# alphafox02/iridium-sniffer

Hardware: AMD Instinct MI355X
Metric: IQ Msamples/s end-to-end (detect->demod), 10 MHz cf32 (higher is better)
Workload: dtype f32

## Files before the change

### iridium-sniffer_amd/csrc/api.cpp

```cpp
#include <stdarg.h>
#include "pipeline.hpp"

namespace irdmh {

extern "C" int irdm_set_option(irdm_pipeline_t *p, const char *key, int value)
{
    if (!p || !key) return -1;
    pipeline_enter(p);
    if (!strcmp(key, "keep_frame_samples")) { p->keep_frame_samples = value; return 0; }
    if (!strcmp(key, "packed_records")) { p->packed_records = value; return 0; }
    if (!strcmp(key, "parsed_records")) { p->parsed_records = value; return 0; }
    if (!strcmp(key, "frame_records")) { p->frame_records = value; return 0; }
    if (!strcmp(key, "chunk_marks")) { p->chunk_marks = value ? 1 : 0; if (!value) p->st.q_marks.clear(); return 0; }
    if (!strcmp(key, "group_member")) { p->in_group = value != 0; return 0; }
    if (!strcmp(key, "spectrum_frames")) {
        if (value < 0 || value > (1 << 20) || p->in_group || p->st.begin_no != 0) return -1;
        return spectrum_configure(p, value);
    }
    if (!strcmp(key, "input_stats")) {
        if (p->in_group || p->st.begin_no != p->st.end_no) return -1;
        return input_stats_configure(p, value);
    }
    if (!strcmp(key, "symbol_clock")) {
        if (p->in_group || p->st.begin_no != p->st.end_no) return -1;
        return symbol_clock_configure(p, value);
    }
    if (!strcmp(key, "decode_frames")) { p->decode_frames = value; return 0; }
    if (!strcmp(key, "decode_ida")) { p->decode_ida = value; return 0; }
    if (!strcmp(key, "detect_only")) { p->detect_only = value; return 0; }
    if (!strcmp(key, "fir_order") || !strcmp(key, "simd_order")) { p->fir_order = value ? 1 : 0; return 0; }
    if (!strcmp(key, "host_cfo")) { p->dev_cfo = p->dev_cfo_ok && value == 0; return 0; }
    if (!strcmp(key, "scan_mode")) { p->scan_mode = value; return 0; }
    if (!strcmp(key, "kernel_clock")) { p->kernel_clock = value != 0; return 0; }
    if (!strcmp(key, "rot_prebuild")) {
        if (value) return p->rot_pre_runs ? 0 : rot_prebuild(p);
        return p->rot_pre_runs ? rot_arena_reset(p, (long long)std::min(p->P.n, 1024) * p->rot_runs) : 0;
    }
    if (!strcmp(key, "band_timeline")) { p->band_tune.timeline = value != 0; return 0; }
    if (!strcmp(key, "fir_generic")) { p->fir_generic = value != 0; return 0; }
    if (!strcmp(key, "post_generic")) { p->post_generic = value != 0; return 0; }
    if (!strcmp(key, "k1_lists")) { p->k1_lists = value; return 0; }
    if (!strcmp(key, "band_first")) { p->band_first = value < 0 ? 0 : value > kBandRounds ? kBandRounds : value; return 0; }
    if (!strcmp(key, "band_spec")) { p->band_spec_opt = value != 0; return 0; }
    if (!strcmp(key, "band_selfcheck")) { p->band_tune.selfcheck = value; return 0; }
    if (!strcmp(key, "rot_pool_rows")) {
        if (value < 1 || value > p->P.n) return -1;
        return rot_arena_reset(p, (long long)value * p->rot_runs);
    }
    if (!strcmp(key, "scratch_outputs")) {
        if (value < 16) return -1;
        for (int i = 0; i < p->n_bc; i++)
            if (p->bc[i].st.n != 0) return -1;
        IRDM_HIP_CHECK(hipDeviceSynchronize());
        for (int i = 0; i < p->n_bc; i++) {
            BatchCtx &b = p->bc[i];
            float2 *d2 = dev_alloc<float2>((size_t)value), *l2 = dev_alloc<float2>(lpf_alloc((size_t)value));
            if (!d2 || !l2) return -1;
            (void)hipFree(b.d_dec);
            (void)hipFree(b.d_lpf);
            b.d_dec = d2;
            b.d_lpf = l2;
            b.dec_cap = (size_t)value;
            if (!b.owns_buffers) { p->d_dec = d2; p->d_lpf = l2; }
// ... 390 lines not shown
```

### iridium-sniffer_amd/csrc/chain.cpp

```cpp
#include "pipeline.hpp"

namespace irdmh {

SampleSource make_source(const irdm_pipeline *p, const void *chunk, uint64_t c0, uint64_t c1)
{
    SampleSource s;
    s.chunk = chunk;
    s.chunk_start = chunk ? c0 : ~0ull;
    s.chunk_end = c1;
    s.ring = p->d_ring;
    s.ring_len = p->ring_len;
    s.ref_ring = p->ref_ring;
    s.fmt = p->dev_fmt;
    s.n_cu = p->n_cu;
    return s;
}

int ring_guard(irdm_pipeline *p, uint64_t a0, uint64_t a1, hipStream_t st)
{
    const uint64_t L = p->ring_len;
    if (a1 <= a0 || L == 0) return 0;
    for (int i = 0; i < p->n_bc; i++) {
        const BatchCtx &b = p->bc[i];
        if (b.st.n <= 0 || b.st.ring_hi <= b.st.ring_lo) continue;
// ... 307 lines not shown
                p->rot_build_gen[(size_t)bin] = p->rot_gen[me] + 1;
            }
    }
    int n_new = 0;
    for (int bin : p->rot_touched) {
        const int from = p->rot_len_h[(size_t)bin], to = p->rot_want[(size_t)bin];
        if (from == 0) p->rot_rows_used++;
        b.hp_rot_new[n_new++] = int4{ bin, from, to, p->rot_blocks_used };
        p->rot_blocks_used += (to - from) / kRotRun;
        p->stat_rot_ckpts += (uint64_t)(to - from);
        p->rot_len_h[(size_t)bin] = to;
        p->rot_want[(size_t)bin] = 0;
        p->rot_build_ctx[(size_t)bin] = me;
        p->rot_build_gen[(size_t)bin] = p->rot_gen[me] + 1;
    }
    p->rot_gen[me]++;
    p->stat_rot_builds++;
    p->stat_rot_rows += (uint64_t)n_new;
    if (launch_copy_words(b.d_rot_new, b.hp_rot_new_dev, sizeof(int4) * (size_t)n_new, st) != 0) return -1;
    if (launch_rotator_rows(p->d_rot_incr, p->d_rot_table, p->rot_runs, b.d_rot_new, n_new, p->d_rot_slot, st) != 0) return -1;
    IRDM_HIP_CHECK(hipEventRecord(b.ev_rot, st));
    return wait_for(wait_mask & ~wait_first);
}

int bursts_enqueue(irdm_pipeline *p, BatchCtx &b, const SampleSource &src, const GoneBurst *gone_list, int nb)
{
    const DetParams &P = p->P;
    const int fs = p->cfg.sample_rate;
    b.st.n = nb;
    b.st.recs.assign(nb, irdm_burst_t());
    size_t n_tiles = 0, dec_need = 0;
    int max_dec_len = 0;
    const int fir_aligned = p->ring_len % 8 == 0 && p->ref_ring % 8 == 0 && (src.chunk_start == ~0ull || src.chunk_start % 8 == 0);
    const int tile_out = fir_tile_out(p->decim, fir_aligned, p->fir_generic, p->fir_order);
    for (int i = 0; i < nb; i++) {
        const GoneBurst &g = gone_list[i];
        irdm_burst_t &r = b.st.recs[i];
        r.id = g.id; r.start = g.start; r.stop = g.stop; r.last_active = g.last_active;
        r.center_bin = g.center_bin;
        r.peak_rel = g.peak_rel; r.base_sum = g.base_sum;
        r.magnitude = 10.0f * log10f(g.peak_rel * kHistory * 1.72f);
        if (r.magnitude > p->st.peak_signal_db) p->st.peak_signal_db = r.magnitude;
        r.noise = 10.0f * log10f(g.base_sum / kHistory / ((float)P.n * P.n) / 1.72f /
                                 ((float)fs / P.n));
        r.num_samples = g.stop + (uint64_t)P.pre_len - g.start;
        uint64_t e = (g.stop + (uint64_t)P.n + p->feed_block - 1) / p->feed_block * p->feed_block;
        r.avail_end = std::min<uint64_t>(e, src.chunk_end);

        BurstWork &w = b.hp_work[i];
        memset(&w, 0, sizeof(w));
        w.start = g.start;
        w.avail_end = r.avail_end;
        w.center_bin = g.center_bin;
        int n = r.num_samples > (uint64_t)(2 * 1024 * 1024) ? 2 * 1024 * 1024 : (int)r.num_samples;
        if ((size_t)n > p->l_cap) {
            fprintf(stderr, "irdm_hip: burst window %d exceeds l_cap %zu\n", n, p->l_cap);
            return -1;
        }
        w.n = n;
        w.dec_len = 0;
        w.drop_reason = 0;
        if (r.num_samples < 100) {
            w.drop_reason = 1;
        } else {
            int n_out = (n - p->in_ntaps + 1) / p->decim;
            if (n_out < 0) n_out = 0;
            w.dec_len = n_out;
            if (n_out < 100) w.drop_reason = 2;
        }
        w.tile_base = (int32_t)n_tiles;
        w.dec_off = (int32_t)dec_need;
        if (!w.drop_reason) {
            max_dec_len = std::max(max_dec_len, w.dec_len);
            n_tiles += (size_t)(w.dec_len + tile_out - 1) / tile_out;
            dec_need += ((size_t)w.dec_len + 15) & ~(size_t)15;
        }
    }
    b.st.ring_lo = b.st.ring_hi = 0;
    if (p->detect_only || nb == 0) return 0;
    {
        uint64_t lo = ~0ull, hi = 0;
        for (int i = 0; i < nb; i++) {
            const BurstWork &w = b.hp_work[i];
            if (w.drop_reason) continue;
            const uint64_t back = w.start + (uint64_t)w.n > w.avail_end ? p->ref_ring : 0;
            lo = std::min(lo, w.start > back ? w.start - back : 0);
            hi = std::max(hi, w.start + (uint64_t)w.n);
        }
        if (lo < hi) { b.st.ring_lo = lo; b.st.ring_hi = hi; }
    }
    if (dec_need > p->stat_scratch_peak) p->stat_scratch_peak = dec_need;
    if (dec_need > b.dec_cap) {
        const size_t cap2 = std::max(dec_need, 2 * b.dec_cap);
        if (cap2 > (size_t)0x7fffffff) {
            fprintf(stderr, "irdm_hip: %zu decimated samples in a batch of %d bursts\n", dec_need, nb);
            return -1;
        }
        float2 *d2 = dev_alloc<float2>(cap2), *l2 = dev_alloc<float2>(lpf_alloc(cap2));
        if (!d2 || !l2) {
            if (d2) (void)hipFree(d2);
            if (l2) (void)hipFree(l2);
            fprintf(stderr, "irdm_hip: no memory for %zu decimated samples per batch\n", cap2);
            return -1;
        }
        p->scratch_retired.push_back(b.d_dec);
        p->scratch_retired.push_back(b.d_lpf);
        b.d_dec = d2;
        b.d_lpf = l2;
        b.dec_cap = cap2;
        if (!b.owns_buffers) { p->d_dec = d2; p->d_lpf = l2; }
        p->stat_scratch_grows++;
    }
    const bool tile_list = fir_needs_tile_list(p->decim, fir_aligned, p->fir_generic) != 0;
    if (n_tiles > b.tiles_cap) {
        if (b.d_tiles) p->tiles_retired.push_back(b.d_tiles);
        if (b.hp_tiles) p->tiles_host_retired.push_back(b.hp_tiles);
        b.hp_tiles = nullptr;
        b.tiles_cap = n_tiles * 2;
        b.d_tiles = dev_alloc<FirTile>((b.tiles_cap + 1) * kFirTileUnits);
        if (!b.owns_buffers) p->d_tiles = b.d_tiles;
        if (!b.d_tiles ||
            hipHostMalloc(reinterpret_cast<void **>(&b.hp_tiles), sizeof(FirTile) * b.tiles_cap, hipHostMallocDefault) != hipSuccess)
            return -1;
        p->stat_tiles_grows++;
    }
    if (tile_list) {
        n_tiles = 0;
        for (int i = 0; i < nb; i++) {
            const BurstWork &w = b.hp_work[i];
            if (!w.drop_reason)
                for (int o = 0; o < w.dec_len; o += tile_out) b.hp_tiles[n_tiles++] = FirTile{ i, o };
        }
    }
    hipStream_t st = b.stream;
    if (rot_rows_prepare(p, b, nb, st) != 0) return -1;
    if (launch_copy_words(b.d_work, b.hp_work_dev, sizeof(BurstWork) * nb, st) != 0) return -1;
    if (tile_list && n_tiles && launch_copy_words(b.d_tiles, b.hp_tiles, sizeof(FirTile) * n_tiles, st) != 0) return -1;
    IRDM_HIP_CHECK(hipEventRecord(b.ev[0], st));
    if (launch_fir_decimate(src, b.d_work, nb, b.d_tiles, b.tiles_cap, (int)n_tiles, p->decim, p->d_in_taps,
                            p->d_fir_off, p->d_rot_incr, p->d_rot_table, p->rot_runs, b.d_dec, st,
                            p->kclk_fir((int)(&b - p->bc)), p->d_rot_slot, p->fir_order, p->fir_generic) != 0)
        return -1;
    IRDM_HIP_CHECK(hipEventRecord(b.ev[1], st));
    if (launch_downmix_post1(b.d_work, nb, max_dec_len, b.d_dec, b.d_lpf, box_of(b.d_lpf, b.dec_cap), p->d_noise_taps,
                             p->noise_ntaps, p->d_start_taps, p->start_ntaps, p->search_depth,
                             p->pre_start, p->d_cfo_window, p->d_tw4096, p->dev_cfo ? nullptr : b.hp_work_dev, st,
                             p->kclk_fir((int)(&b - p->bc)), p->fir_order, p->post_generic) != 0)
        return -1;
    CfoStep cfo;
    cfo.on_device = p->dev_cfo ? 1 : 0;
    cfo.n_fft = P.n;
    cfo.sample_rate = fs;
    cfo.out_rate = p->out_rate;
    cfo.center_frequency = p->cfg.center_frequency;
    b.cfo_on_device = p->dev_cfo;
    if (!p->dev_cfo) {
        IRDM_HIP_CHECK(hipEventRecord(b.ev_cfo, st));
        b.cfo_seq++;
        {
            std::lock_guard<std::mutex> lk(p->cfo_mu);
            p->cfo_jobs.push_back(&b);
        }
        p->cfo_cv.notify_one();
        if (launch_wait_host_flag(b.hp_flag_dev, b.cfo_seq, b.hp_flag_dev + 1, st) != 0) return -1;
    }
    if (launch_downmix_post2(b.d_work, nb, b.d_lpf, p->d_rrc_taps, p->rrc_ntaps,
                             p->d_tw2048, p->d_dl_fft, p->d_ul_fft, p->dl_len, p->ul_len, p->sps,
                             b.d_rrc_ws, b.d_frames, p->dev_cfo ? nullptr : b.hp_work_dev, cfo, st, p->fir_order, p->post_generic) != 0)
        return -1;
    IRDM_HIP_CHECK(hipEventRecord(b.ev[2], st));
    b.packed = (p->packed_records || p->parsed_records || p->frame_records) && !p->decode_frames && !p->decode_ida &&
               !p->keep_frame_samples;
    b.parsed = b.packed && p->parsed_records;
    b.framed = b.packed && p->frame_records;
// ... 218 lines not shown
```

### iridium-sniffer_amd/csrc/downmix.hip

```cpp
#include <algorithm>
#include <cstdio>
#include "common.hpp"
#include "types.hpp"
#include "kernels.hpp"
#include "burst_src.hpp"
#include "libm_port.hpp"

namespace irdm {

#include "fir_fma.inc"

__global__ void rotator_rows_kernel(const float2 *__restrict__ incr, float2 *__restrict__ table, int n_runs,
                                    const int4 *__restrict__ news, int n_new, int *__restrict__ runs_all)
{
    const int i = blockIdx.x * blockDim.x + threadIdx.x;
    if (i >= n_new) return;
    const int bin = news[i].x, from = news[i].y, to = news[i].z, block0 = news[i].w;
    const float2 inc = incr[bin];
    int *runs = runs_all + (size_t)bin * n_runs;
    float2 ph = make_float2(1.0f, 0.0f);
    if (from > 0) {
        ph = table[(size_t)runs[(from - 1) / kRotRun] * kRotRun + (from - 1) % kRotRun];
#pragma unroll
        for (int u = 0; u < kRotSeg; u++) ph = cmul(ph, inc);
// ... 175 lines not shown
    g.avail_end = w->avail_end;
    g.ring_pos = g.a_tile % ring_len;
    const int cb = w->center_bin;
    const float2 inc = rot_incr[cb];
    g.inc_re = inc.x;
    g.inc_im = inc.y;
    {
        const int c0 = g.s0 / kRotSeg, r0 = c0 / kRotRun;
        const int *runs = rot_slot + (size_t)cb * n_ckpt;
        const int b0 = runs[r0];
        int b1 = r0 + 1 < n_ckpt ? runs[r0 + 1] : b0;
        if (b1 < 0) b1 = b0;
        g.ck_index = (uint64_t)b0 * kRotRun + (uint64_t)(c0 % kRotRun);
        g.ck_wrap = kRotRun - c0 % kRotRun;
        g.ck_index2 = (uint64_t)b1 * kRotRun;
    }
    g.out_base = (int64_t)w->dec_off + o0;
    g.stale_pos = (g.ring_pos + ring_len - ref_ring % ring_len) % ring_len;
    g.pad = 0;
    geom[t] = g;
}

int fir_tile_row(int decim)
{
    int r = kFirTileOut + kFirTaps / decim + 2;
    while ((r & 15) != 1) r++;
    return r;
}

static bool fir_reg_path(int decim, int aligned, int generic) { return !generic && aligned && fir_reg_supported(decim); }

int fir_needs_tile_list(int decim, int aligned, int generic) { return fir_reg_path(decim, aligned, generic) ? 0 : 1; }

int fir_tile_out(int decim, int aligned, int generic, int order)
{
    if (!fir_reg_path(decim, aligned, generic)) return kFirTileOut;
    return order ? fir_fma_tile_out(decim) : fir_reg_tile_out(decim);
}

int launch_fir_decimate(const SampleSource &src, const BurstWork *work, int n_bursts, FirTile *tiles, size_t tiles_cap,
                        int n_tiles, int decim, const float *taps, const int *tap_off, const float2 *rot_incr,
                        const float2 *rot_table, int n_ckpt, float2 *dec,
                        hipStream_t stream, unsigned long long *kclk, const int *rot_slot, int order, int generic)
{
    if (n_tiles <= 0) return 0;
    const int aligned = src.ring_len % 8 == 0 && src.ref_ring % 8 == 0 && (src.chunk_start == ~0ull || src.chunk_start % 8 == 0);
    if (fir_reg_path(decim, aligned, generic) && tiles_cap >= (size_t)n_tiles) {
        FirGeom *geom = reinterpret_cast<FirGeom *>(tiles + tiles_cap);
        hipLaunchKernelGGL(fir_geom_kernel, dim3((n_tiles + 255) / 256), dim3(256), 0, stream, work, n_bursts, n_tiles, decim,
                           order ? fir_fma_tile_out(decim) : fir_reg_tile_out(decim), src.ring_len, src.ref_ring, rot_incr, n_ckpt,
                           geom, rot_slot);
        return (order ? launch_fir_fma(src, geom, n_tiles, decim, taps, rot_table, dec, stream, kclk)
                      : launch_fir_reg(src, geom, n_tiles, decim, taps, rot_table, dec, stream, kclk)) == 0 ? 0 : -1;
    }
    const int row = fir_tile_row(decim);
    const size_t lds = sizeof(float2) * (size_t)row * decim;
    if (lds > 160 * 1024) return -1;
    (void)hipFuncSetAttribute((const void *)fir_decimate_kernel,
                              hipFuncAttributeMaxDynamicSharedMemorySize, (int)lds);
    hipLaunchKernelGGL(fir_decimate_kernel, dim3(n_tiles), dim3(kFirTileOut), lds, stream, src, work,
                       tiles, decim, row, taps, tap_off, rot_incr, rot_table, n_ckpt, dec, order, rot_slot);
    return hipGetLastError() == hipSuccess ? 0 : -1;
}

__global__ void copy_words_kernel(uint32_t *__restrict__ dst, const uint32_t *__restrict__ src, size_t n)
{
    for (size_t i = blockIdx.x * (size_t)blockDim.x + threadIdx.x; i < n; i += (size_t)gridDim.x * blockDim.x)
        __hip_atomic_store(dst + i, __hip_atomic_load(src + i, __ATOMIC_RELAXED, __HIP_MEMORY_SCOPE_SYSTEM),
                           __ATOMIC_RELAXED, __HIP_MEMORY_SCOPE_SYSTEM);
    __threadfence_system();
}

__global__ void gone_export_kernel(const DetState *__restrict__ st, const uint32_t *__restrict__ gone, int cap,
                                   uint32_t *__restrict__ hp_gone, uint32_t *__restrict__ hp_hdr,
                                   const uint32_t *__restrict__ ctl, uint32_t *__restrict__ hp_ctl, int ctl_words)
{
    gone_export_body(st, gone, cap, hp_gone, hp_hdr, ctl, hp_ctl, ctl_words, (int)gridDim.x);
}

int launch_gone_export(const DetState *st, const GoneBurst *gone, int cap, GoneBurst *hp_gone, uint32_t *hp_hdr,
                       const void *ctl, void *hp_ctl, int ctl_bytes, hipStream_t stream)
{
    hipLaunchKernelGGL(gone_export_kernel, dim3(32), dim3(256), 0, stream, st, reinterpret_cast<const uint32_t *>(gone), cap,
// ... 744 lines not shown
```

### iridium-sniffer_amd/csrc/fir_reg.hip

```cpp
#include <cstdio>
#include "common.hpp"
#include "types.hpp"
#include "kernels.hpp"
#include "burst_src.hpp"

#ifndef IRDM_FIR_KCLK
#define IRDM_FIR_KCLK 1
#endif

namespace irdm {

#include "fir_mac.inc"

constexpr int kFirStrip = 3;

template <int M>
struct FirR {
    static constexpr int NR = kFirTaps / M;
    static constexpr int REM = kFirTaps - NR * M;
    static_assert(M % 8 == 0 && NR < 63 && REM >= 1, "geometry");
};

int fir_reg_supported(int decim) { return decim == 40 || decim == 48; }

// ... 220 lines not shown
            __builtin_amdgcn_sched_barrier(0);
            mac_rest(tb, H);
        }
        shift();
        {
            constexpr int P0 = REM >= H ? H : 0;
            if constexpr (REM >= H) {
                mac_head(ta, 0);
                mac_rest(ta, 0);
            }
            const uint64_t *t = taps64 + (NR * M + P0) / 2;
#pragma unroll
            for (int gq = 0; gq < (REM - P0) / 8; gq++)
                fir_mac2x8(acc[0], acc[1], &y[0][P0 + 8 * gq], &y[1][P0 + 8 * gq], t + 4 * gq);
#pragma unroll
            for (int p = P0 + (REM - P0) / 8 * 8; p < REM; p++) {
                const float tq = taps[NR * M + p];
                acc[0] = acc[0] + y[0][p] * tq;
                acc[1] = acc[1] + y[1][p] * tq;
            }
        }
#pragma unroll
        for (int j = 0; j < 2; j++) {
            const int q = 128 * d + 64 * j + lane - NR;
            if (q >= 0 && q < g.n_out) dec[g.out_base + q] = make_float2(acc[j].x, acc[j].y);
        }
    }
    }
    if (IRDM_FIR_KCLK) kclk_leave(kclk);
}

#include "fir_fma.inc"

int fir_fma_tile_out(int decim) { return 128 - kFirTaps / decim; }

template <int M, int FMT>
__device__ __forceinline__ void fir_fetch_column(const SampleSource &src, const FirGeom &g, int cr, int n_cols, v2f *y)
{
    const bool needed = cr < n_cols;
    const int k0 = needed ? cr * M : 0;
    const uint64_t a0 = g.a_tile + (uint64_t)k0;
    uint64_t rp = g.ring_pos + (uint64_t)k0;
    if (rp >= src.ring_len) rp -= src.ring_len;
    const bool in_chunk = a0 >= src.chunk_start;
    const bool simple = a0 + M <= g.avail_end && (in_chunk || (a0 + M <= src.chunk_start && rp + M <= src.ring_len));
    if (__builtin_amdgcn_ballot_w64(needed && !simple) == 0) {
        const void *base = in_chunk ? src.chunk : src.ring;
        const size_t idx = !needed ? 0 : in_chunk ? (size_t)(a0 - src.chunk_start) : (size_t)rp;
#pragma unroll
        for (int i = 0; i < M / 8; i++) load_piece<FMT>(base, idx + 8 * i, &y[8 * i]);
    } else {
        uint64_t rs = g.stale_pos + (uint64_t)k0;
        if (rs >= src.ring_len) rs -= src.ring_len;
#pragma unroll
        for (int i = 0; i < M / 8; i++) {
            const uint64_t a = a0 + 8 * i;
            v2f xn[8], xs[8];
#pragma unroll
            for (int u = 0; u < 8; u++) xn[u] = xs[u] = v2f{ 0.0f, 0.0f };
            if (needed && a < g.avail_end) {
                uint64_t p = rp + 8 * i;
                if (p >= src.ring_len) p -= src.ring_len;
                if (a >= src.chunk_start) load_piece<FMT>(src.chunk, (size_t)(a - src.chunk_start), xn);
                else load_piece<FMT>(src.ring, (size_t)p, xn);
            }
            if (needed && a + 8 > g.avail_end && a >= src.ref_ring) {
                const uint64_t as = a - src.ref_ring;
                uint64_t p = rs + 8 * i;
                if (p >= src.ring_len) p -= src.ring_len;
                if (as >= src.chunk_start) load_piece<FMT>(src.chunk, (size_t)(as - src.chunk_start), xs);
                else load_piece<FMT>(src.ring, (size_t)p, xs);
            }
#pragma unroll
            for (int u = 0; u < 8; u++) y[8 * i + u] = (a + u < g.avail_end) ? xn[u] : xs[u];
        }
    }
}

template <int M, int FMT>
__global__ __launch_bounds__(64) __attribute__((amdgpu_waves_per_eu(2, 2))) void fir_decimate_kernel_f(
    SampleSource src, const FirGeom *__restrict__ geom, const float *__restrict__ taps,
    const float2 *__restrict__ rot_table, float2 *__restrict__ dec, int n_tiles, unsigned long long *__restrict__ kclk)
{
    using R = FirR<M>;
    constexpr int NR = R::NR, REM = R::REM;
    constexpr int VT = REM - 1;
    static_assert(NR % 2 == 0, "rows are unrolled in pairs (the accumulator sets swap names)");
    static_assert(M % 4 == 0 && VT % 8 == 0 && (kFirTaps - 1) % 4 == 0, "tap k -> accumulator k % 4 = (k % M) % 4; one tap left over");
    const int lane = threadIdx.x;
    kclk_enter(kclk);
#pragma unroll 1
    for (int tile = blockIdx.x; tile < n_tiles;) {
        const int tile_next = tile + (int)gridDim.x;
        const FirGeom g = geom[tile];
        tile = tile_next;
        const int n_cols = g.n_out + NR;
        const v2f inc = { g.inc_re, g.inc_im };
        const uint64_t *taps64 = reinterpret_cast<const uint64_t *>(taps);
        v2f y[2][M];
#pragma unroll
        for (int j = 0; j < 2; j++) fir_fetch_column<M, FMT>(src, g, 2 * lane + j, n_cols, y[j]);
        {
            v2f ph[2];
#pragma unroll
            for (int j = 0; j < 2; j++) {
                const int cr = 2 * lane + j;
                const int k0 = cr < n_cols ? cr * M : 0;
                const float2 c = rot_table[fir_ck(g, k0 / kRotSeg)];
                ph[j] = v2f{ c.x, c.y };
            }
            if (M % kRotSeg != 0) {
                static_assert(M % kRotSeg == 0 || M % kRotSeg == 8, "a column starts on a checkpoint or 8 samples behind one");
                v2f pw = ph[1];
#pragma unroll
                for (int u = 0; u < 8; u++) pw = cmul_pk(pw, inc);
                if (2 * lane + 1 < n_cols) ph[1] = pw;
            }
#pragma unroll
            for (int p = 0; p < M; p++) {
                v2f r0, r1, n0, n1;
                cmul_pk2(r0, y[0][p], ph[0], r1, y[1][p], ph[1]);
                cmul_pk2(n0, ph[0], inc, n1, ph[1], inc);
                y[0][p] = r0;
                y[1][p] = r1;
                ph[0] = n0;
                ph[1] = n1;
            }
        }
        const v2f zero = { 0.0f, 0.0f };
        v2f X[4] = { zero, zero, zero, zero }, Y[4] = { zero, zero, zero, zero };
        constexpr int H = M / 2;
        static_assert(H == 20 || H == 24, "half rows of 8 + 8 + 4 or 8 + 8 + 8 taps");
        uint64_t ta[H / 2], tb[H / 2];
        auto request = [&](uint64_t (&t)[H / 2], int tap0) {
#pragma unroll
            for (int i = 0; i < H / 2; i++) t[i] = taps64[tap0 / 2 + i];
        };
        auto half_rest = [&](v2f (&xa)[4], v2f (&xb)[4], const uint64_t *t, int p0) {
            fir_fma2x8(xa, xb, &y[0][p0 + 8], &y[1][p0 + 8], t + 4);
            if constexpr (H == 24) fir_fma2x8(xa, xb, &y[0][p0 + 16], &y[1][p0 + 16], t + 8);
            else fir_fma2x4(xa, xb, &y[0][p0 + 16], &y[1][p0 + 16], t + 8);
        };
        auto row = [&](v2f (&xa)[4], v2f (&xb)[4], int r, int next_tap0) {
            fir_fma2x8(xa, xb, &y[0][0], &y[1][0], ta);
            __builtin_amdgcn_sched_barrier(0);
            request(tb, r * M + H);
            __builtin_amdgcn_sched_barrier(0);
            half_rest(xa, xb, ta, 0);
            fir_fma2x8(xa, xb, &y[0][H], &y[1][H], tb);
            __builtin_amdgcn_sched_barrier(0);
            request(ta, next_tap0);
            __builtin_amdgcn_sched_barrier(0);
            half_rest(xa, xb, tb, H);
        };
        auto shift = [&](v2f (&x)[4]) {
#pragma unroll
            for (int j = 0; j < 4; j++) {
                x[j].x = lane_shr1(x[j].x);
                x[j].y = lane_shr1(x[j].y);
            }
        };
        request(ta, 0);
#pragma unroll 1
        for (int rp = 0; rp < NR / 2; rp++) {
            row(X, Y, 2 * rp, (2 * rp + 1) * M);
            shift(Y);
            row(Y, X, 2 * rp + 1, (2 * rp + 2 < NR || VT >= H) ? (2 * rp + 2) * M : 0);
            shift(X);
        }
        if constexpr (VT > 0) {
            static_assert(VT < H || VT == H + 8, "VT = 32 at M = 48");
            if constexpr (VT >= H) {
                fir_fma2x8(X, Y, &y[0][0], &y[1][0], ta);
                half_rest(X, Y, ta, 0);
                const uint64_t *t = taps64 + (NR * M + H) / 2;
                fir_fma2x8(X, Y, &y[0][H], &y[1][H], t);
            } else {
                const uint64_t *t = taps64 + (NR * M) / 2;
#pragma unroll
                for (int gq = 0; gq < VT / 8; gq++) fir_fma2x8(X, Y, &y[0][8 * gq], &y[1][8 * gq], t + 4 * gq);
            }
        }
        {
            const float tq = taps[kFirTaps - 1];
            const v2f sa = (X[0] + X[2]) + (X[1] + X[3]), sb = (Y[0] + Y[2]) + (Y[1] + Y[3]);
            const v2f oa = sa + y[0][VT] * tq, ob = sb + y[1][VT] * tq;
            const int qa = 2 * lane - NR, qb = qa + 1;
            if (qa >= 0 && qa < g.n_out) dec[g.out_base + qa] = make_float2(oa.x, oa.y);
            if (qb >= 0 && qb < g.n_out) dec[g.out_base + qb] = make_float2(ob.x, ob.y);
        }
    }
    kclk_leave(kclk);
}

template <int M>
static int launch_fir_f_fmt(const SampleSource &src, const FirGeom *geom, int n_tiles, const float *taps,
                            const float2 *rot_table, float2 *dec, hipStream_t stream, unsigned long long *kclk)
{
    const int n_cu = src.n_cu > 0 ? src.n_cu : 256;
    const int grid = 7 * n_cu < n_tiles ? 7 * n_cu : n_tiles;
    if (src.fmt == 2) hipLaunchKernelGGL((fir_decimate_kernel_f<M, 2>), dim3(grid), dim3(64), 0, stream, src, geom, taps, rot_table, dec, n_tiles, kclk);
    else if (src.fmt == 1) hipLaunchKernelGGL((fir_decimate_kernel_f<M, 1>), dim3(grid), dim3(64), 0, stream, src, geom, taps, rot_table, dec, n_tiles, kclk);
    else if (src.fmt == 3) hipLaunchKernelGGL((fir_decimate_kernel_f<M, 3>), dim3(grid), dim3(64), 0, stream, src, geom, taps, rot_table, dec, n_tiles, kclk);
    else if (src.fmt == 4) hipLaunchKernelGGL((fir_decimate_kernel_f<M, 4>), dim3(grid), dim3(64), 0, stream, src, geom, taps, rot_table, dec, n_tiles, kclk);
    else if (src.fmt == 0) hipLaunchKernelGGL((fir_decimate_kernel_f<M, 0>), dim3(grid), dim3(64), 0, stream, src, geom, taps, rot_table, dec, n_tiles, kclk);
    else if (src.fmt == 6) hipLaunchKernelGGL((fir_decimate_kernel_f<M, 6>), dim3(grid), dim3(64), 0, stream, src, geom, taps, rot_table, dec, n_tiles, kclk);
    else if (src.fmt == 8) hipLaunchKernelGGL((fir_decimate_kernel_f<M, 8>), dim3(grid), dim3(64), 0, stream, src, geom, taps, rot_table, dec, n_tiles, kclk);
    else if (src.fmt == 9) hipLaunchKernelGGL((fir_decimate_kernel_f<M, 9>), dim3(grid), dim3(64), 0, stream, src, geom, taps, rot_table, dec, n_tiles, kclk);
    else return -1;
    return hipGetLastError() == hipSuccess ? 0 : -1;
}

int launch_fir_fma(const SampleSource &src, const FirGeom *geom, int n_tiles, int decim, const float *taps,
                   const float2 *rot_table, float2 *dec, hipStream_t stream, unsigned long long *kclk)
{
    if (src.ring_len % 8 != 0 || src.ref_ring % 8 != 0 || (src.chunk_start != ~0ull && src.chunk_start % 8 != 0)) return 1;
    switch (decim) {
    case 40: return launch_fir_f_fmt<40>(src, geom, n_tiles, taps, rot_table, dec, stream, kclk);
    case 48: return launch_fir_f_fmt<48>(src, geom, n_tiles, taps, rot_table, dec, stream, kclk);
    default: return 1;
    }
}
// ... 34 lines not shown
```

### iridium-sniffer_amd/csrc/kernels.hpp

```cpp
#pragma once
#include <hip/hip_runtime.h>
#include <vector>
#include "types.hpp"

namespace irdm {

int launch_fft_mag_lists(int log_n, int fmt, const void *iq, const float *window, const float2 *tw, float *mag,
                         int n_frames, const float *pre, unsigned *counts, ListEntry *entries, int cap,
                         hipStream_t stream, unsigned long long *kclk, int order);
int launch_prefilter_threshold(const float *sum, float thr, float *pre, int n, hipStream_t stream);
int launch_fft_mag(int log_n, int fmt, const void *iq, const float *window, const float2 *tw,
                   float *mag, int n_frames, hipStream_t stream, unsigned long long *kclk, int order);
int launch_detect_scan(const DetParams &P, DetState *st, float *sum, float *hist, const float *mag,
                       int n_frames, GoneBurst *gone, int gone_cap, PeakCand *cand_a,
                       PeakCand *cand_b, hipStream_t stream);

struct ZeroRegions {
    static constexpr int kMax = 8;
    uint32_t *ptr[kMax];
    uint32_t words[kMax];
    int n = 0;
    bool add(void *p, size_t bytes)
    {
        if (!p || n >= kMax || bytes % 4 != 0 || bytes / 4 > 0xffffffffull) return false;
// ... 67 lines not shown
    int sum_restart = 1;
};
int band_list_cap(int n);
int band_scan_supported(const DetParams &D, BandParams *out, int n_frames, uint64_t idx0);
size_t band_work_bytes(int n, size_t max_chunk, bool spec = false);
int band_work_carve(BandWork *W, void *base, int n, size_t max_chunk, bool spec = false);
int launch_band_spec(const DetParams &D, BandWork S, DetState *st_spec, const float *sum_src, int n_frames, uint64_t idx0,
                     const unsigned *counts, const ListEntry *entries, int have_prev, hipStream_t stream, const BandTune &tune);
int launch_band_scan(const DetParams &D, BandWork W, DetState *st, float *sum, float *hist, const float *mag,
                     int n_frames, uint64_t idx0, const unsigned *counts, const ListEntry *entries, const float *pre,
                     float *smin, GoneBurst *gone, int gone_cap, int round_begin, int round_end, GoneBurst *hp_gone,
                     uint32_t *hp_hdr, void *hp_ctl, int hp_cap, int chained, int tl_sel, hipStream_t stream,
                     const BandTune &tune, const uint32_t *gate_flag = nullptr, uint32_t gate_seq = 0, uint32_t *gate_err = nullptr,
                     const void *gate_src = nullptr, size_t gate_bytes = 0,
                     const BandWork *spec = nullptr, hipEvent_t sums_done = nullptr);
constexpr int kBandTlSlots = 32;
int launch_prefilter_lists(const float *sum, float thr, float *pre, const float *smin, const float *mag, int n,
                           unsigned *counts, ListEntry *entries, int n_frames, int cap, hipStream_t stream);

struct SampleSource {
    const void *chunk;
    uint64_t chunk_start;
    uint64_t chunk_end;
    const void *ring;
    uint64_t ring_len;
    uint64_t ref_ring;
    int fmt;
    int n_cu;
};

int launch_rotator_rows(const float2 *incr, float2 *table, int n_runs, const int4 *news, int n_new, int *runs, hipStream_t stream);
int fir_tile_row(int decim);
int fir_reg_supported(int decim);
int fir_fma_tile_out(int decim);
int fir_reg_tile_out(int decim);
int launch_fir_fma(const SampleSource &src, const FirGeom *geom, int n_tiles, int decim, const float *taps,
                   const float2 *rot_table, float2 *dec, hipStream_t stream, unsigned long long *kclk = nullptr);
int launch_fir_reg(const SampleSource &src, const FirGeom *geom, int n_tiles, int decim, const float *taps,
                   const float2 *rot_table, float2 *dec, hipStream_t stream, unsigned long long *kclk = nullptr);
int fir_tile_out(int decim, int aligned, int generic, int order);
int fir_needs_tile_list(int decim, int aligned, int generic);
int launch_fir_decimate(const SampleSource &src, const BurstWork *work, int n_bursts, FirTile *tiles, size_t tiles_cap,
                        int n_tiles, int decim, const float *taps, const int *tap_off, const float2 *rot_incr,
                        const float2 *rot_table, int n_ckpt, float2 *dec,
                        hipStream_t stream, unsigned long long *kclk,
                        const int *rot_slot, int order, int generic);
int launch_kclk_fold(unsigned long long *kclk, hipStream_t stream);
int launch_gone_export(const DetState *st, const GoneBurst *gone, int cap, GoneBurst *hp_gone, uint32_t *hp_hdr,
                       const void *ctl, void *hp_ctl, int ctl_bytes, hipStream_t stream);
int launch_copy_to_host(void *dst, const void *src, size_t bytes, hipStream_t stream);
int launch_copy2_to_host(void *dst_a, const void *src_a, size_t bytes_a, void *dst_b, const void *src_b, size_t bytes_b,
                         hipStream_t stream);
int launch_copy_words(void *dst, const void *src, size_t bytes, hipStream_t stream);
int launch_wait_host_flag(const uint32_t *flag, uint32_t seq, uint32_t *err, hipStream_t stream);
int launch_gather_burst(const SampleSource &src, uint64_t start, uint64_t avail_end, int n,
                        float2 *out, hipStream_t stream);
int launch_downmix_post1(BurstWork *work, int n_bursts, int max_dec_len, float2 *dec,
                         float2 *lpf, float *box, const float *noise_taps, int noise_ntaps,
                         const float *start_taps, int start_ntaps, int search_depth, int pre_start,
                         const float *cfo_window, const float2 *tw4096, BurstWork *hp_work, hipStream_t stream,
                         unsigned long long *kclk,
                         int order, int generic);
struct CfoStep {
    int on_device;
    int n_fft, sample_rate, out_rate;
    double center_frequency;
};
int launch_downmix_post2(BurstWork *work, int n_bursts, const float2 *lpf,
                         const float *rrc_taps, int rrc_ntaps, const float2 *tw2048,
                         const float2 *dl_fft, const float2 *ul_fft, int dl_len, int ul_len,
                         float sps, float2 *rrc_ws, float2 *frames, const BurstWork *hp_work, const CfoStep &cfo,
                         hipStream_t stream, int order, int generic);
int launch_sincosf_probe(const float *x, size_t n, float *re, float *im, hipStream_t stream);

int launch_ida_decode(const DemodOut *frames, int n_frames, const int2 *syn_da, const int2 *syn_l1, const int2 *syn_l2,
                      const int2 *syn_l3, int use_llr, const int *n_bits, const int *direction, IdaOut *out,
                      hipStream_t stream);
int launch_frame_decode(const DemodOut *frames, int n_frames, const int2 *syn_ra, const int2 *syn_hdr, int use_llr,
                        const int *n_bits, DecodedOut *out, hipStream_t stream);
// ... 46 lines not shown
```

### iridium-sniffer_amd/csrc/pipeline.hpp

```cpp
#pragma once
#include <math.h>
#include <stdlib.h>
#include <string.h>
#include <time.h>
#include <errno.h>
#include <sys/stat.h>
#include <algorithm>
#include <deque>
#include <new>
#include <vector>
#include <thread>
#include <mutex>
#include <condition_variable>
#include "../../include/irdm_hip.h"
#include "common.hpp"
#include "host_design.hpp"
#include "kernels.hpp"
#include "libm_port.hpp"
#include "band_core.hpp"
#include "types.hpp"
#include "record_queues.hpp"
#include "input_stats.hpp"
#include "symbol_clock.hpp"

// ... 149 lines not shown

struct irdm_pipeline {
    irdm_config_t cfg;
    StreamState st;
    DetParams P;
    int dev_fmt;
    size_t bps;
    int feed_block, decim, out_rate;
    bool dev_cfo;
    bool dev_cfo_ok;
    float sps;
    uint64_t ref_ring, ring_len;
    size_t l_cap;
    int n_ckpt, dec_stride, burst_cap, gone_cap;
    size_t max_chunk;
    int search_depth, pre_start;
    int in_ntaps, noise_ntaps, start_ntaps, rrc_ntaps, dl_len, ul_len;

    hipStream_t stream;
    hipStream_t bstream;
    hipStream_t stream2;
    int bstream_prio;
    hipStream_t sstream;
    hipEvent_t ev_scan_in, ev_scan_out;
    int band_spec_opt = 1;
    void *d_band_spec = nullptr;
    BandWork band_spec = {};
    DetState *d_state_spec = nullptr;
    hipStream_t stream_spec = nullptr;
    hipEvent_t ev_sums1 = nullptr;
    hipEvent_t ev_spec_done = nullptr;
    uint64_t stat_spec_passes = 0, stat_spec_scans = 0, stat_sum_restarts = 0;
    int fir_order = 1;
    int fir_generic = 0;
    int post_generic = 0;
    irdm::BandTune band_tune;
    hipEvent_t ev[10];

    float *d_window, *d_hist, *d_sum, *d_mag;
    float2 *d_tw, *d_tw4096, *d_tw2048, *d_dl_fft, *d_ul_fft, *d_rot_incr, *d_rot_table;
    DetState *d_state;
    GoneBurst *d_gone;
    PeakCand *d_cand_a, *d_cand_b;
    void *d_ring, *d_stage;
    float *d_in_taps, *d_noise_taps, *d_start_taps, *d_rrc_taps, *d_cfo_window;
    int *d_fir_off;
    BurstWork *d_work;
    FirTile *d_tiles;
    size_t tiles_cap;
    float2 *d_dec, *d_lpf, *d_rrc_ws, *d_frames, *d_demod_ws, *d_probe;
    DemodOut *d_demod;
    DecodedOut *d_decoded;
    int2 *d_syn_ra, *d_syn_hdr;
    int *d_nbits;
    int decode_frames, decode_ida, detect_only;
    IdaOut *d_ida;
    int2 *d_syn_da, *d_syn_l1, *d_syn_l2, *d_syn_l3;
    int *d_dirs;
    std::vector<IdaOut> h_ida;
    std::vector<DecodedOut> h_decoded;
    unsigned *d_counts, *d_goff;
    ListEntry *d_entries, *d_compact;
    float *d_pre, *d_sum_bak, *d_hist_bak;
    DetState *d_state_bak;
    int *d_status;
    unsigned long long *d_mc_ops;
// ... 151 lines not shown
```

Before: 77040.

## Process multi-block FIR strips per tile with LDS carry and host-side strip-size selection

The FMA FIR decimation kernel can now process a tile as a strip of up to four 128-column blocks in sequence. The lane-shift carry across block boundaries goes through shared memory, so the tap overhang (kFirTaps/decim) is paid once per strip instead of once per block. On the host, the strip size (1..4) is picked by simulating the per-workgroup load over the persistent grid for each candidate and keeping the one with the smallest makespan. The row loop is also unrolled by two. In exchange it adds shared-memory traffic and a wave barrier per row, longer serial work per tile, and host-side cost for the selection loop.

After: 79160, median of 6. 1.03x the previous value.

```diff
diff --git a/iridium-sniffer_amd/csrc/api.cpp b/iridium-sniffer_amd/csrc/api.cpp
--- a/iridium-sniffer_amd/csrc/api.cpp
+++ b/iridium-sniffer_amd/csrc/api.cpp
@@ -29,6 +29,11 @@
     if (!strcmp(key, "decode_ida")) { p->decode_ida = value; return 0; }
     if (!strcmp(key, "detect_only")) { p->detect_only = value; return 0; }
     if (!strcmp(key, "fir_order") || !strcmp(key, "simd_order")) { p->fir_order = value ? 1 : 0; return 0; }
+    if (!strcmp(key, "fir_strip")) {
+        if (value < 0 || value > kFirStripMax) return -1;
+        p->fir_strip = value;
+        return 0;
+    }
     if (!strcmp(key, "host_cfo")) { p->dev_cfo = p->dev_cfo_ok && value == 0; return 0; }
     if (!strcmp(key, "scan_mode")) { p->scan_mode = value; return 0; }
     if (!strcmp(key, "kernel_clock")) { p->kernel_clock = value != 0; return 0; }
diff --git a/iridium-sniffer_amd/csrc/chain.cpp b/iridium-sniffer_amd/csrc/chain.cpp
--- a/iridium-sniffer_amd/csrc/chain.cpp
+++ b/iridium-sniffer_amd/csrc/chain.cpp
@@ -363,7 +363,6 @@
     size_t n_tiles = 0, dec_need = 0;
     int max_dec_len = 0;
     const int fir_aligned = p->ring_len % 8 == 0 && p->ref_ring % 8 == 0 && (src.chunk_start == ~0ull || src.chunk_start % 8 == 0);
-    const int tile_out = fir_tile_out(p->decim, fir_aligned, p->fir_generic, p->fir_order);
     for (int i = 0; i < nb; i++) {
         const GoneBurst &g = gone_list[i];
         irdm_burst_t &r = b.st.recs[i];
@@ -399,13 +398,52 @@
             w.dec_len = n_out;
             if (n_out < 100) w.drop_reason = 2;
         }
-        w.tile_base = (int32_t)n_tiles;
         w.dec_off = (int32_t)dec_need;
         if (!w.drop_reason) {
             max_dec_len = std::max(max_dec_len, w.dec_len);
-            n_tiles += (size_t)(w.dec_len + tile_out - 1) / tile_out;
             dec_need += ((size_t)w.dec_len + 15) & ~(size_t)15;
         }
+    }
+    int fir_strip = 1;
+    if (fir_strip_choice(p->decim, fir_aligned, p->fir_generic, p->fir_order)) {
+        fir_strip = p->fir_strip;
+        if (!fir_strip) {
+            const size_t grid = 7 * (size_t)(src.n_cu > 0 ? src.n_cu : 256);
+            std::vector<int64_t> load(grid + 1);
+            int64_t best = 0;
+            for (int s = 1; s <= kFirStripMax; s++) {
+                const size_t t = (size_t)fir_tile_out(p->decim, fir_aligned, p->fir_generic, p->fir_order, s);
+                const size_t nr = 128 * (size_t)s - t;
+                std::fill(load.begin(), load.end(), 0);
+                int64_t laps = 0;
+                size_t tile = 0;
+                for (int i = 0; i < nb; i++) {
+                    const BurstWork &w = b.hp_work[i];
+                    if (w.drop_reason || w.dec_len <= 0) continue;
+                    const size_t n = ((size_t)w.dec_len + t - 1) / t, full = n - 1;
+                    laps += (int64_t)(full / grid) * s;
+                    const size_t w0 = tile % grid, rest = full % grid;
+                    load[w0] += s;
+                    if (w0 + rest <= grid) load[w0 + rest] -= s;
+                    else { load[grid] -= s; load[0] += s; load[w0 + rest - grid] -= s; }
+                    const size_t wl = (tile + full) % grid;
+                    const int64_t bl = (int64_t)(((size_t)w.dec_len - full * t + nr + 127) / 128);
+                    load[wl] += bl;
+                    load[wl + 1] -= bl;
+                    tile += n;
+                }
+                int64_t sum = 0, cost = 0;
+                for (size_t k = 0; k < grid; k++) { sum += load[k]; cost = std::max(cost, sum); }
+                cost += laps;
+                if (s == 1 || cost < best) { best = cost; fir_strip = s; }
+            }
+        }
+    }
+    const int tile_out = fir_tile_out(p->decim, fir_aligned, p->fir_generic, p->fir_order, fir_strip);
+    for (int i = 0; i < nb; i++) {
+        BurstWork &w = b.hp_work[i];
+        w.tile_base = (int32_t)n_tiles;
+        if (!w.drop_reason) n_tiles += (size_t)(w.dec_len + tile_out - 1) / tile_out;
     }
     b.st.ring_lo = b.st.ring_hi = 0;
     if (p->detect_only || nb == 0) return 0;
@@ -470,7 +508,7 @@
     IRDM_HIP_CHECK(hipEventRecord(b.ev[0], st));
     if (launch_fir_decimate(src, b.d_work, nb, b.d_tiles, b.tiles_cap, (int)n_tiles, p->decim, p->d_in_taps,
                             p->d_fir_off, p->d_rot_incr, p->d_rot_table, p->rot_runs, b.d_dec, st,
-                            p->kclk_fir((int)(&b - p->bc)), p->d_rot_slot, p->fir_order, p->fir_generic) != 0)
+                            p->kclk_fir((int)(&b - p->bc)), p->d_rot_slot, p->fir_order, p->fir_generic, fir_strip) != 0)
         return -1;
     IRDM_HIP_CHECK(hipEventRecord(b.ev[1], st));
     if (launch_downmix_post1(b.d_work, nb, max_dec_len, b.d_dec, b.d_lpf, box_of(b.d_lpf, b.dec_cap), p->d_noise_taps,
diff --git a/iridium-sniffer_amd/csrc/downmix.hip b/iridium-sniffer_amd/csrc/downmix.hip
--- a/iridium-sniffer_amd/csrc/downmix.hip
+++ b/iridium-sniffer_amd/csrc/downmix.hip
@@ -231,23 +231,26 @@
 
 int fir_needs_tile_list(int decim, int aligned, int generic) { return fir_reg_path(decim, aligned, generic) ? 0 : 1; }
 
-int fir_tile_out(int decim, int aligned, int generic, int order)
+int fir_tile_out(int decim, int aligned, int generic, int order, int strip)
 {
     if (!fir_reg_path(decim, aligned, generic)) return kFirTileOut;
-    return order ? fir_fma_tile_out(decim) : fir_reg_tile_out(decim);
-}
+    return order ? fir_fma_tile_out(decim, strip) : fir_reg_tile_out(decim);
+}
+
+int fir_strip_choice(int decim, int aligned, int generic, int order) { return fir_reg_path(decim, aligned, generic) && order ? 1 : 0; }
 
 int launch_fir_decimate(const SampleSource &src, const BurstWork *work, int n_bursts, FirTile *tiles, size_t tiles_cap,
                         int n_tiles, int decim, const float *taps, const int *tap_off, const float2 *rot_incr,
                         const float2 *rot_table, int n_ckpt, float2 *dec,
-                        hipStream_t stream, unsigned long long *kclk, const int *rot_slot, int order, int generic)
+                        hipStream_t stream, unsigned long long *kclk, const int *rot_slot, int order, int generic, int strip)
 {
     if (n_tiles <= 0) return 0;
+    if (strip < 1 || strip > kFirStripMax) return -1;
     const int aligned = src.ring_len % 8 == 0 && src.ref_ring % 8 == 0 && (src.chunk_start == ~0ull || src.chunk_start % 8 == 0);
     if (fir_reg_path(decim, aligned, generic) && tiles_cap >= (size_t)n_tiles) {
         FirGeom *geom = reinterpret_cast<FirGeom *>(tiles + tiles_cap);
         hipLaunchKernelGGL(fir_geom_kernel, dim3((n_tiles + 255) / 256), dim3(256), 0, stream, work, n_bursts, n_tiles, decim,
-                           order ? fir_fma_tile_out(decim) : fir_reg_tile_out(decim), src.ring_len, src.ref_ring, rot_incr, n_ckpt,
+                           order ? fir_fma_tile_out(decim, strip) : fir_reg_tile_out(decim), src.ring_len, src.ref_ring, rot_incr, n_ckpt,
                            geom, rot_slot);
         return (order ? launch_fir_fma(src, geom, n_tiles, decim, taps, rot_table, dec, stream, kclk)
                       : launch_fir_reg(src, geom, n_tiles, decim, taps, rot_table, dec, stream, kclk)) == 0 ? 0 : -1;
diff --git a/iridium-sniffer_amd/csrc/fir_reg.hip b/iridium-sniffer_amd/csrc/fir_reg.hip
--- a/iridium-sniffer_amd/csrc/fir_reg.hip
+++ b/iridium-sniffer_amd/csrc/fir_reg.hip
@@ -276,7 +276,12 @@
 
 #include "fir_fma.inc"
 
-int fir_fma_tile_out(int decim) { return 128 - kFirTaps / decim; }
+int fir_fma_tile_out(int decim, int blocks) { return 128 * blocks - kFirTaps / decim; }
+
+__device__ __forceinline__ float lane_shr1_old(float old, float v)
+{
+    return __int_as_float(__builtin_amdgcn_update_dpp(__float_as_int(old), __float_as_int(v), 0x138 , 0xf, 0xf, false));
+}
 
 template <int M, int FMT>
 __device__ __forceinline__ void fir_fetch_column(const SampleSource &src, const FirGeom &g, int cr, int n_cols, v2f *y)
@@ -331,24 +336,34 @@
     constexpr int VT = REM - 1;
     static_assert(NR % 2 == 0, "rows are unrolled in pairs (the accumulator sets swap names)");
     static_assert(M % 4 == 0 && VT % 8 == 0 && (kFirTaps - 1) % 4 == 0, "tap k -> accumulator k % 4 = (k % M) % 4; one tap left over");
+    static_assert(128 * kFirStripMax * M <= kRotRun * kRotSeg, "a strip crosses at most one checkpoint-run boundary");
     const int lane = threadIdx.x;
     kclk_enter(kclk);
+    __shared__ __attribute__((aligned(16))) v2f s_carry[NR][4];
+    const v2f zero = { 0.0f, 0.0f };
+    for (int i = lane; i < NR * 4; i += 64) s_carry[i >> 2][i & 3] = zero;
+    __builtin_amdgcn_fence(__ATOMIC_RELEASE, "wavefront");
+    __builtin_amdgcn_wave_barrier();
 #pragma unroll 1
     for (int tile = blockIdx.x; tile < n_tiles;) {
         const int tile_next = tile + (int)gridDim.x;
         const FirGeom g = geom[tile];
         tile = tile_next;
         const int n_cols = g.n_out + NR;
+        const int n_blk = (n_cols + 127) >> 7;
         const v2f inc = { g.inc_re, g.inc_im };
         const uint64_t *taps64 = reinterpret_cast<const uint64_t *>(taps);
+#pragma unroll 1
+        for (int d = 0; d < n_blk; d++) {
+        const int c0 = 128 * d + 2 * lane;
         v2f y[2][M];
 #pragma unroll
-        for (int j = 0; j < 2; j++) fir_fetch_column<M, FMT>(src, g, 2 * lane + j, n_cols, y[j]);
+        for (int j = 0; j < 2; j++) fir_fetch_column<M, FMT>(src, g, c0 + j, n_cols, y[j]);
         {
             v2f ph[2];
 #pragma unroll
             for (int j = 0; j < 2; j++) {
-                const int cr = 2 * lane + j;
+                const int cr = c0 + j;
                 const int k0 = cr < n_cols ? cr * M : 0;
                 const float2 c = rot_table[fir_ck(g, k0 / kRotSeg)];
                 ph[j] = v2f{ c.x, c.y };
@@ -358,7 +373,7 @@
                 v2f pw = ph[1];
 #pragma unroll
                 for (int u = 0; u < 8; u++) pw = cmul_pk(pw, inc);
-                if (2 * lane + 1 < n_cols) ph[1] = pw;
+                if (c0 + 1 < n_cols) ph[1] = pw;
             }
 #pragma unroll
             for (int p = 0; p < M; p++) {
@@ -371,7 +386,6 @@
                 ph[1] = n1;
             }
         }
-        const v2f zero = { 0.0f, 0.0f };
         v2f X[4] = { zero, zero, zero, zero }, Y[4] = { zero, zero, zero, zero };
         constexpr int H = M / 2;
         static_assert(H == 20 || H == 24, "half rows of 8 + 8 + 4 or 8 + 8 + 8 taps");
@@ -385,7 +399,7 @@
             if constexpr (H == 24) fir_fma2x8(xa, xb, &y[0][p0 + 16], &y[1][p0 + 16], t + 8);
             else fir_fma2x4(xa, xb, &y[0][p0 + 16], &y[1][p0 + 16], t + 8);
         };
-        auto row = [&](v2f (&xa)[4], v2f (&xb)[4], int r, int next_tap0) {
+        auto row = [&](v2f (&xa)[4], v2f (&xb)[4], v2f (&cin)[4], int r, int next_tap0) {
             fir_fma2x8(xa, xb, &y[0][0], &y[1][0], ta);
             __builtin_amdgcn_sched_barrier(0);
             request(tb, r * M + H);
@@ -394,23 +408,34 @@
             fir_fma2x8(xa, xb, &y[0][H], &y[1][H], tb);
             __builtin_amdgcn_sched_barrier(0);
             request(ta, next_tap0);
+#pragma unroll
+            for (int j = 0; j < 4; j++) cin[j] = s_carry[r][j];
             __builtin_amdgcn_sched_barrier(0);
             half_rest(xa, xb, tb, H);
         };
-        auto shift = [&](v2f (&x)[4]) {
+        auto shift = [&](v2f (&x)[4], const v2f (&cin)[4], int r) {
+            const v2f x0[4] = { x[0], x[1], x[2], x[3] };
 #pragma unroll
             for (int j = 0; j < 4; j++) {
-                x[j].x = lane_shr1(x[j].x);
-                x[j].y = lane_shr1(x[j].y);
+                x[j].x = lane_shr1_old(cin[j].x, x0[j].x);
+                x[j].y = lane_shr1_old(cin[j].y, x0[j].y);
+            }
+            __builtin_amdgcn_fence(__ATOMIC_ACQ_REL, "wavefront");
+            __builtin_amdgcn_wave_barrier();
+            if (lane == 63) {
+#pragma unroll
+                for (int j = 0; j < 4; j++) s_carry[r][j] = x0[j];
             }
         };
         request(ta, 0);
-#pragma unroll 1
+        static_assert(NR % 4 == 0, "row pairs are unrolled in pairs");
+#pragma unroll 2
         for (int rp = 0; rp < NR / 2; rp++) {
-            row(X, Y, 2 * rp, (2 * rp + 1) * M);
-            shift(Y);
-            row(Y, X, 2 * rp + 1, (2 * rp + 2 < NR || VT >= H) ? (2 * rp + 2) * M : 0);
-            shift(X);
+            v2f cin[4];
+            row(X, Y, cin, 2 * rp, (2 * rp + 1) * M);
+            shift(Y, cin, 2 * rp);
+            row(Y, X, cin, 2 * rp + 1, (2 * rp + 2 < NR || VT >= H) ? (2 * rp + 2) * M : 0);
+            shift(X, cin, 2 * rp + 1);
         }
         if constexpr (VT > 0) {
             static_assert(VT < H || VT == H + 8, "VT = 32 at M = 48");
@@ -429,9 +454,10 @@
             const float tq = taps[kFirTaps - 1];
             const v2f sa = (X[0] + X[2]) + (X[1] + X[3]), sb = (Y[0] + Y[2]) + (Y[1] + Y[3]);
             const v2f oa = sa + y[0][VT] * tq, ob = sb + y[1][VT] * tq;
-            const int qa = 2 * lane - NR, qb = qa + 1;
+            const int qa = c0 - NR, qb = qa + 1;
             if (qa >= 0 && qa < g.n_out) dec[g.out_base + qa] = make_float2(oa.x, oa.y);
             if (qb >= 0 && qb < g.n_out) dec[g.out_base + qb] = make_float2(ob.x, ob.y);
+        }
         }
     }
     kclk_leave(kclk);
diff --git a/iridium-sniffer_amd/csrc/kernels.hpp b/iridium-sniffer_amd/csrc/kernels.hpp
--- a/iridium-sniffer_amd/csrc/kernels.hpp
+++ b/iridium-sniffer_amd/csrc/kernels.hpp
@@ -123,19 +123,22 @@
 int launch_rotator_rows(const float2 *incr, float2 *table, int n_runs, const int4 *news, int n_new, int *runs, hipStream_t stream);
 int fir_tile_row(int decim);
 int fir_reg_supported(int decim);
-int fir_fma_tile_out(int decim);
+int fir_fma_tile_out(int decim, int blocks);
+constexpr int kFirStripMax = 4;
 int fir_reg_tile_out(int decim);
 int launch_fir_fma(const SampleSource &src, const FirGeom *geom, int n_tiles, int decim, const float *taps,
                    const float2 *rot_table, float2 *dec, hipStream_t stream, unsigned long long *kclk = nullptr);
 int launch_fir_reg(const SampleSource &src, const FirGeom *geom, int n_tiles, int decim, const float *taps,
                    const float2 *rot_table, float2 *dec, hipStream_t stream, unsigned long long *kclk = nullptr);
-int fir_tile_out(int decim, int aligned, int generic, int order);
+int fir_tile_out(int decim, int aligned, int generic, int order, int strip);
+int fir_strip_choice(int decim, int aligned, int generic, int order);
 int fir_needs_tile_list(int decim, int aligned, int generic);
 int launch_fir_decimate(const SampleSource &src, const BurstWork *work, int n_bursts, FirTile *tiles, size_t tiles_cap,
                         int n_tiles, int decim, const float *taps, const int *tap_off, const float2 *rot_incr,
                         const float2 *rot_table, int n_ckpt, float2 *dec,
                         hipStream_t stream, unsigned long long *kclk,
-                        const int *rot_slot, int order, int generic);
+                        const int *rot_slot, int order, int generic,
+                        int strip);
 int launch_kclk_fold(unsigned long long *kclk, hipStream_t stream);
 int launch_gone_export(const DetState *st, const GoneBurst *gone, int cap, GoneBurst *hp_gone, uint32_t *hp_hdr,
                        const void *ctl, void *hp_ctl, int ctl_bytes, hipStream_t stream);
diff --git a/iridium-sniffer_amd/csrc/pipeline.hpp b/iridium-sniffer_amd/csrc/pipeline.hpp
--- a/iridium-sniffer_amd/csrc/pipeline.hpp
+++ b/iridium-sniffer_amd/csrc/pipeline.hpp
@@ -205,6 +205,7 @@
     hipEvent_t ev_spec_done = nullptr;
     uint64_t stat_spec_passes = 0, stat_spec_scans = 0, stat_sum_restarts = 0;
     int fir_order = 1;
+    int fir_strip = 0;
     int fir_generic = 0;
     int post_generic = 0;
     irdm::BandTune band_tune;
```
